# rst-tu-dortmund/mpc_local_planner

Measured on AMD Instinct MI355X. Metric: MPC solves/sec (batched control cycles) at N=50 carlike, higher is better.
Workload: dtype f64

## Files before the change

### mpc_local_planner_amd/csrc/mpc_wave.hpp

```cpp
#pragma once
#include <hip/hip_runtime.h>
#include <type_traits>

#include "mpc_core.hpp"
#include "mpc_dpp_blocks.inc"

#include "mpc_wave_debug.hpp"
#include "mpc_wave_layout.hpp"

namespace mpc {

template <typename T, int MODEL, int EXT = 1, bool OBST = true, int NSC = 0, bool GS = false, bool W2 = false, int SHAPE = 0>
struct IpmWave {
    static constexpr int NSTG = EXT ? NSTG_EXT : NSTG_BASE;
    static constexpr int NTRB = (MODEL == MODEL_KINEMATIC_BICYCLE || MODEL == MODEL_SIMPLE_CAR_FRONT) ? 4 : 3;
    static_assert(NSC == 0 || (EXT == 0 && !OBST), "the fixed layout exists for the headline instantiation only");
    static_assert(!GS || NSC == 0, "the fixed layout keeps its factorisation data in LDS");
    static_assert(!W2 || (!GS && EXT == 0 && !OBST), "the two-wave kernel exists for the headline instantiation in the LDS form only");
    static_assert(SHAPE == 0 || NSC != 0, "a compile-time shape exists for the fixed layout only");
    using LayoutT = typename LayoutOf<NSC, NTRB, NSTG>::type;
    const Problem<T>& P;
    const LayoutT L;
    T* sm;
    T* gmb = nullptr;
    const int lane;
    T x0[3], xf[3], uprev[2], dtprev;
    T mu, rho, delta_last;
    T erho = T(0);
    bool row0_on, fail0;
    bool warm_guess = false;
    mutable int cnt_mult = -1, cnt_bmult = -1;
    mutable T inv_cnt_mult = T(1), inv_cnt_bmult = T(1);
    int nvia = 0;
    int flags;
    MPC_PROF_MEMBERS
    int nfix;
    int my_cand = 0, iter_cap = 0;
    int rows_dropped = 0;
    const double* dual_in = nullptr;
    const int* win_ptr = nullptr;

    __device__ IpmWave(const Problem<T>& p, const WaveLayout& l, T* s, int ln) : P(p), L(LayoutOf<NSC, NTRB, NSTG>::from(l)), sm(s), lane(ln) {}

    __device__ __forceinline__ T& F(int base, int comp, int k) const { return sm[base + comp * L.NS + k]; }
    typedef __attribute__((address_space(1))) T GlbT;
    typedef __attribute__((address_space(1))) char GlbC;
    using SwT = std::conditional_t<GS, GlbT, T>;
    __device__ __forceinline__ GlbT& gw(unsigned word) const { return *(GlbT*)((GlbC*)gmb + (size_t)(word * (unsigned)sizeof(T))); }
    static constexpr int TE_CC = NSTG, TE_Z = NSTG + 3, TNT = GlobalStage::nt(NSTG);
    __device__ __forceinline__ int tile_k(int k) const { return GlobalStage::TILE(L.NS) + ((k + GlobalStage::kGuard) >> 2) * (4 * TNT) + ((k + GlobalStage::kGuard) & 3); }
    __device__ __forceinline__ GlbT& TL_(int e, int k) const { return gw((unsigned)(tile_k(k) + 4 * e)); }
    __device__ __forceinline__ SwT& G_(int i, int k) const { if constexpr (GS) return gw((unsigned)(GlobalStage::GAIN + k * NGAIN + i)); else return sm[L.GAIN + k * NGAIN + i]; }
    static constexpr int NADDv = EXT ? (int)NADD : (int)NADD_BASE;
    __device__ __forceinline__ SwT& S_(int i, int k) const { if constexpr (GS) return TL_(i, k); else return sm[L.STG + k * NSTG + i]; }
    __device__ __forceinline__ T& C_(int i, int k) const { return sm[L.CC + k * 3 + i]; }
    __device__ __forceinline__ SwT& OB_(int which, int m, int k) const {
        if constexpr (GS) return gw((unsigned)(GlobalStage::OBC(L.NS, NSTG) + (which * L.M + m) * L.NS + k)); else return sm[(which == 0 ? L.OG : (which == 1 ? L.OAX : (which == 2 ? L.OAY : L.OHK))) + m * L.NS + k];
    }
    __device__ __forceinline__ SwT& OX_(int which, int m, int k) const {
        if constexpr (GS) return gw((unsigned)(L.OXB + ((which < 4 ? which * L.MT : 4 * L.MT + (which - 4) * L.MD) + m) * L.NS + k));
        else {
            const int base = which == 0 ? L.OAT : (which == 1 ? L.OHXT : (which == 2 ? L.OHYT : (which == 3 ? L.OHTT : (which == 4 ? L.OAD : (which == 5 ? L.OHXD : (which == 6 ? L.OHYD : (which == 7 ? L.OHDD : L.OHTD)))))));
            return sm[base + m * L.NS + k];
        }
    }
    __device__ __forceinline__ GlbT& OE_(int which, int m, int k) const { return gw((unsigned)(L.OEB + (which * L.M + m) * L.NS + k)); }
    __device__ __forceinline__ T& CH_(int i, int k) const { return sm[L.LAMN + i * L.NS + k]; }
    __device__ __forceinline__ T& SCL(int i) const { return sm[L.SC + i]; }
    __device__ __forceinline__ void sync() const { __syncthreads(); }
    __device__ __forceinline__ int nM() const { return OBST ? L.M : 0; }
    __device__ __forceinline__ unsigned short* oi_base() const { return reinterpret_cast<unsigned short*>(sm + L.OI); }
    __device__ __forceinline__ int oi(int m, int k) const { const unsigned v = oi_base()[m * L.NS + k]; return v == 0xffffu ? -1 : (int)v; }
    __device__ __forceinline__ void set_oi(int m, int k, int j) const { oi_base()[m * L.NS + k] = (unsigned short)(j < 0 ? 0xffff : j); }
    __device__ __forceinline__ bool fx(int i) const { if constexpr (SHAPE != 0) return (SHAPE >> i) & 1; else return (flags >> i) & 1; }
    __device__ __forceinline__ bool dtf() const { if constexpr (SHAPE != 0) return (SHAPE >> 3) & 1; else return (flags >> 3) & 1; }
    __device__ __forceinline__ bool dtf_sum() const { return (flags >> 3) & 1; }
    __device__ __forceinline__ bool quad() const { if constexpr (SHAPE != 0) return (SHAPE >> 4) & 1; else return (flags >> 4) & 1; }
    __device__ __forceinline__ bool hasqf() const { if constexpr (SHAPE != 0) return (SHAPE >> 5) & 1; else return (flags >> 5) & 1; }
    __device__ __forceinline__ bool mintime() const { if constexpr (SHAPE != 0) return (SHAPE >> 16) & 1; else return (flags >> 16) & 1; }
    __device__ __forceinline__ bool costx() const { return EXT >= 2; }
    __device__ __forceinline__ void offmul(const T o[3], const T x[3], T y[3]) const {
        y[0] = o[0] * x[1] + o[1] * x[2]; y[1] = o[0] * x[0] + o[2] * x[2]; y[2] = o[1] * x[0] + o[2] * x[1];
    }
    __device__ __forceinline__ T offquad(const T o[3], const T x[3]) const { return T(2) * (o[0] * x[0] * x[1] + o[1] * x[0] * x[2] + o[2] * x[1] * x[2]); }
    __device__ __forceinline__ T fullquad(const T dg[3], const T o[3], const T x[3]) const { return dg[0] * x[0] * x[0] + dg[1] * x[1] * x[1] + dg[2] * x[2] * x[2] + offquad(o, x); }
    __device__ __forceinline__ void xd_final(T alpha, T xd[3]) const {
        for (int i = 0; i < 3; ++i) { xd[i] = fx(i) ? T(0) : xt(i, L.n - 1, alpha) - xf[i]; }
        xd[2] = normalize_theta(xd[2]);
    }
    __device__ __forceinline__ T final_cost_extra(T alpha, T d) const {
        T xd[3]; xd_final(alpha, xd);
        T f = T(0);
        if (hasqf()) f += offquad(P.Qfo, xd);
        if (P.trapz) f += T(0.5) * d * fullquad(P.Q, P.Qo, xd);
        return f;
    }
    __device__ __forceinline__ bool ron(int q) const { if constexpr (SHAPE != 0) return (SHAPE >> (6 + q)) & 1; else return (flags >> (6 + q)) & 1; }
    __device__ __forceinline__ bool ball() const { return EXT && ((flags >> 10) & 1); }
    __device__ __forceinline__ bool via() const { return EXT && ((flags >> 11) & 1); }
    __device__ __forceinline__ bool fpline() const { return EXT && ((flags >> 12) & 1); }
    __device__ __forceinline__ bool intf() const { return EXT && ((flags >> 13) & 1); }
    __device__ __forceinline__ bool dynobs() const { return EXT && ((flags >> 14) & 1); }
    __device__ __forceinline__ bool hessm() const { return EXT && ((flags >> 15) & 1); }
    typedef __attribute__((address_space(3))) T LdsT;
    __device__ __forceinline__ LdsT* lds(int word) const { return (LdsT*)sm + word; }
    typedef __attribute__((address_space(3))) char LdsC;
    __device__ __forceinline__ LdsT* ldsb(unsigned bytes) const { return (LdsT*)((LdsC*)(LdsT*)sm + bytes); }
    __device__ __forceinline__ static LdsT* lds_adv(LdsT* p, int bytes) { return (LdsT*)((LdsC*)p + bytes); }
    __device__ __forceinline__ static const LdsT* lds_adv(const LdsT* p, int bytes) { return (const LdsT*)((const LdsC*)p + bytes); }
    using SwRef = std::conditional_t<GS, unsigned, LdsT*>;
    using SwCRef = std::conditional_t<GS, unsigned, const LdsT*>;
    __device__ __forceinline__ int W_ZC() const { if constexpr (GS) return GlobalStage::ZC; else return L.ZC; }
    __device__ __forceinline__ int STG_W(int i) const { return L.STG + i; }
    __device__ __forceinline__ int GAIN_W(int i) const { if constexpr (GS) return GlobalStage::GAIN + i; else return L.GAIN + i; }
    __device__ __forceinline__ int CC_W(int i) const { return L.CC + i; }
    __device__ __forceinline__ int CH_W(int i) const { return L.LAMN + i * L.NS; }
    static constexpr int STG_S = NSTG, GAIN_S = NGAIN, CC_S = 3;
    __device__ __forceinline__ int ZT_W(int kind) const { return L.ZC + (kind == 1 ? 4 : (kind == 2 ? 3 : 0)); }
    __device__ __forceinline__ static constexpr int zt_entry(int kind) { return TE_Z + (kind == 1 ? 3 : (kind == 2 ? 2 : 0)); }
    __device__ __forceinline__ int GAIN_DUMMY_W() const { if constexpr (GS) return GlobalStage::GAIN + L.NS * NGAIN; else return L.VP; }
    __device__ __forceinline__ T gld(unsigned stage_bytes, unsigned lane_bytes) const { return *(const GlbT*)((const GlbC*)gmb + (size_t)stage_bytes + (size_t)lane_bytes); }
    __device__ __forceinline__ SwRef sw(int word) const { if constexpr (GS) return (unsigned)word * (unsigned)sizeof(T); else return lds(word); }
    __device__ __forceinline__ static constexpr int sw_step(int words) { return GS ? words * (int)sizeof(T) : words; }
    __device__ __forceinline__ T sw_ld(SwCRef p, int i = 0) const { if constexpr (GS) return *(const GlbT*)((const GlbC*)gmb + (size_t)p + (size_t)(i * (int)sizeof(T))); else return p[i]; }
    __device__ __forceinline__ T sw_ld_at(SwCRef p, int step) const { if constexpr (GS) return *(const GlbT*)((const GlbC*)gmb + (size_t)(p + (unsigned)step)); else return p[step]; }
    __device__ __forceinline__ void sw_st(SwRef p, int i, T v) const { if constexpr (GS) *(GlbT*)((GlbC*)gmb + (size_t)p + (size_t)(i * (int)sizeof(T))) = v; else p[i] = v; }

    static constexpr bool kLocalLiterals = NSC != 0 && sizeof(T) == 8;
    static constexpr bool LL = kLocalLiterals;
    int colloc_ = 0;
    __device__ __forceinline__ int colloc() const { if constexpr (kLocalLiterals) return colloc_; else return P.collocation; }
    __device__ __forceinline__ T normalize_theta(T th) const { return mpc::normalize_theta<kLocalLiterals>(th); }
    using LogAccT = LogAcc<T, kLocalLiterals>;

    __device__ __forceinline__ T xt(int i, int k, T alpha) const {
        T x = F(L.X, i, k);
        if (alpha != T(0) && k > 0 && (k < L.n - 1 || !fx(i))) { x += alpha * F(L.DX, i, k); if (i == 2) x = normalize_theta(x); }
        return x;
    }
    __device__ __forceinline__ T ut(int j, int k, T alpha) const {
        T u = F(L.U, j, k);
        if (alpha != T(0)) u += alpha * F(L.DU, j, k);
        return u;
    }

    __device__ __forceinline__ bool row_on(int r, int q) const { return ron(q) && (r > 0 || row0_on); }

    __device__ __forceinline__ T row_val(int UB, T d, int r, int q) const {
        const int n = L.n, j = q & 1;
        T ur = r < n - 1 ? F(UB, j, r) : T(0);
        const T up0 = uprev[0], up1 = uprev[1];
        T um = j ? up1 : up0;
        if (r > 0) um = F(UB, j, r - 1);
        T dtp = r > 0 ? d : dtprev;
        return slot_sign<T>(q) * ((ur - um) - P.rate_lim[q] * dtp);
    }
    __device__ __forceinline__ T row_jdz(int r, int q, T dd) const {
        const int n = L.n, j = q & 1;
        T dur = r < n - 1 ? F(L.DU, j, r) : T(0);
        T dum = r > 0 ? F(L.DU, j, r - 1) : T(0);
        return slot_sign<T>(q) * ((dur - dum) - (r > 0 ? P.rate_lim[q] * dd : T(0)));
    }

    __device__ __forceinline__ T push_interior(T v, T lb, T ub) const {
        T pl = t_min(Algo<T>::bound_push * t_max(T(1), t_abs(lb)), Algo<T>::bound_push * (ub - lb));
        T pu = t_min(Algo<T>::bound_push * t_max(T(1), t_abs(ub)), Algo<T>::bound_push * (ub - lb));
        return t_min(t_max(v, lb + pl), ub - pu);
    }

    __device__ __forceinline__ int local_lane() const { int l = lane; asm volatile("" : "+v"(l)); return l; }
#define MPC_PHASE_LANE const int lane = W2 ? this->local_lane() : this->lane; (void)lane;
    static constexpr bool kUniformScalars = W2 || (EXT == 0 && !OBST && !GS);
    __device__ __forceinline__ static double uni_(double v) { return __hiloint2double(__builtin_amdgcn_readfirstlane(__double2hiint(v)), __builtin_amdgcn_readfirstlane(__double2loint(v))); }
    __device__ __forceinline__ static float uni_(float v) { return __int_as_float(__builtin_amdgcn_readfirstlane(__float_as_int(v))); }
    __device__ __forceinline__ static int uni_(int v) { return __builtin_amdgcn_readfirstlane(v); }
    __device__ __forceinline__ static long long uni_(long long v) { return ((long long)__builtin_amdgcn_readfirstlane((int)(v >> 32)) << 32) | (unsigned)__builtin_amdgcn_readfirstlane((int)v); }
    __device__ __attribute__((noinline)) static T pow_cold(T a, T b) { return t_pow(a, b); }
    __device__ __forceinline__ static T pow_(T a, T b) { if constexpr (W2 || kLocalLiterals) return pow_cold(a, b); else return t_pow(a, b); }
    __device__ __forceinline__ static void U(T& v) { if constexpr (kUniformScalars) v = uni_(v); }
    template <typename... Ts> __device__ __forceinline__ static void U(T& v, Ts&... rest) { U(v); U(rest...); }

#include "mpc_wave_rows.inc"
#include "mpc_wave_passes.inc"
#include "mpc_wave_sweeps.inc"
#include "mpc_wave_pit.inc"
#include "mpc_wave_step.inc"
#include "mpc_wave_solve.inc"
#undef MPC_PHASE_LANE
};

}
```

### mpc_local_planner_amd/csrc/mpc_wave_step.inc

```

    struct Fwd { T hdz, clam, dz2, dphi, a_p, a_d, dzmax, nunu; bool finite; };

    __device__ __forceinline__ void ftb_ratio(T ival, T dval, T& r) const { r = t_max(r, -dval * ival); }
    __device__ __forceinline__ T ftb_alpha(T r, T tau) const { return r > tau ? tau / r : T(1); }

    template <bool REC>
    __device__ __forceinline__ Fwd post_pass(T dd, const T nu[3], T tau, TrialRegs& tr) const {
        MPC_PHASE_LANE
        const int n = L.n;
        const T d = SCL(SC_D);
        T hdz = T(0), clam = T(0), dz2 = T(0), dphi = T(0), r_p = T(0), r_d = T(0), dzmax = T(0);
        if constexpr (REC) {
            trial_setup_states(tr, lane);
            for (int j = 0; j < 2; ++j) { tr.ulb[j] = P.u_lb[j]; tr.uub[j] = P.u_ub[j]; tr.u[j] = tr.du[j] = T(0); }
            for (int q = 0; q < 4; ++q) { tr.on[q] = false; tr.s[q] = T(1); tr.ds[q] = T(0); }
        }
        if (lane == 0) {
            if (dtf()) {
                T dl = d - P.dt_lb, du = P.dt_ub - d;
                T pl = SCL(SC_PDL), pu = SCL(SC_PDU);
                const T idl = t_rcp(dl), idu = t_rcp(du);
                T gb = -mu * idl + mu * idu;
                hdz += gb * dd; dphi += gb * dd;
                ftb_ratio(idl, dd, r_p); ftb_ratio(idu, -dd, r_p);
                ftb_ratio(t_rcp(pl), mu * idl - pl - (pl * idl) * dd, r_d);
                ftb_ratio(t_rcp(pu), mu * idu - pu + (pu * idu) * dd, r_d);
                dz2 += dd * dd; dzmax = t_max(dzmax, t_abs(dd));
            }
            if (mintime()) { hdz += T(n - 1) * dd; dphi += T(n - 1) * dd; }
            if (ball()) {
                const T jdz = ball_jdz(), s = SCL(SC_TS), y = SCL(SC_TY), res = SCL(SC_TG) + s;
                const T is = t_rcp(s);
                const T sig = y * is, ybar = mu * is + sig * res;
                const T ds = -res - jdz, dy = ybar + sig * jdz - y;
                hdz += ybar * jdz;
                dphi -= (mu * is) * ds;
                ftb_ratio(is, ds, r_p);
                ftb_ratio(t_rcp(y), dy, r_d);
            }
        }
        for (int k = lane; k < n; k += kWave) {
            if (k < n - 1) {
                for (int j = 0; j < 2; ++j) {
                    T u = F(L.U, j, k), du_ = F(L.DU, j, k);
                    T dl = u - P.u_lb[j], du = P.u_ub[j] - u;
                    T pl = F(L.PL, j, k), pu = F(L.PU, j, k);
                    const T idl = t_rcp(dl), idu = t_rcp(du);
                    T gbar = mu * idu - mu * idl + (quad() ? T(2) * P.R[j] * u * (intf() ? d : T(1)) : T(0));
                    if (costx() && quad()) gbar += T(2) * P.Ro * F(L.U, 1 - j, k) * (intf() ? d : T(1));
                    hdz += gbar * du_; dphi += gbar * du_;
                    ftb_ratio(idl, du_, r_p); ftb_ratio(idu, -du_, r_p);
                    ftb_ratio(t_rcp(pl), mu * idl - pl - (pl * idl) * du_, r_d);
                    ftb_ratio(t_rcp(pu), mu * idu - pu + (pu * idu) * du_, r_d);
                    dz2 += du_ * du_; dzmax = t_max(dzmax, t_abs(du_));
                    if constexpr (REC) { tr.u[j] = u; tr.du[j] = du_; }
                }
                for (int i = 0; i < 3; ++i) {
                    clam += C_(i, k) * F(L.LAMN, i, k);
                }
                if (intf()) {
                    const T xd0 = F(L.X, 0, k) - xf[0], xd1 = F(L.X, 1, k) - xf[1], xd2 = normalize_theta(F(L.X, 2, k) - xf[2]);
                    const T v = F(L.U, 0, k), w = F(L.U, 1, k);
                    T sc = P.Q[0] * xd0 * xd0 + P.Q[1] * xd1 * xd1 + P.Q[2] * xd2 * xd2 + P.R[0] * v * v + P.R[1] * w * w;
                    if (costx()) {
                        const T xd[3] = {xd0, xd1, xd2};
                        sc += offquad(P.Qo, xd) + T(2) * P.Ro * v * w;
                        if (k == 0 && P.trapz) sc -= T(0.5) * fullquad(P.Q, P.Qo, xd);
                    }
                    hdz += sc * dd; dphi += sc * dd;
                }
            }
            if (k >= 1) {
                T vg[3] = {T(0), T(0), T(0)};
                if (via() && k < n - 1) { T vv; via_terms(k, F(L.X, 0, k), F(L.X, 1, k), F(L.X, 2, k), vv, vg); }
                T gxo[3] = {T(0), T(0), T(0)};
                if (costx()) {
                    if (k < n - 1) {
                        if (quad()) {
                            const T xd[3] = {F(L.X, 0, k) - xf[0], F(L.X, 1, k) - xf[1], normalize_theta(F(L.X, 2, k) - xf[2])};
                            offmul(P.Qo, xd, gxo);
                            for (int i = 0; i < 3; ++i) gxo[i] *= T(2) * (intf() ? d : T(1));
                        }
                    } else {
                        T xdT[3], y3[3]; xd_final(T(0), xdT);
                        if (hasqf()) { offmul(P.Qfo, xdT, y3); for (int i = 0; i < 3; ++i) gxo[i] += T(2) * y3[i]; }
                        if (P.trapz) {
                            offmul(P.Qo, xdT, y3);
                            for (int i = 0; i < 3; ++i) gxo[i] += d * (P.Q[i] * xdT[i] + y3[i]);
                            const T sc = T(0.5) * fullquad(P.Q, P.Qo, xdT);
                            hdz += sc * dd; dphi += sc * dd;
                        }
                    }
                }
                for (int i = 0; i < 3; ++i) {
                    if (k < n - 1 || !fx(i)) {
                        T dx = F(L.DX, i, k);
                        dz2 += dx * dx; dzmax = t_max(dzmax, t_abs(dx));
                        T g = vg[i];
                        if (quad() && k < n - 1) { T xd = F(L.X, i, k) - xf[i]; if (i == 2) xd = normalize_theta(xd); g = T(2) * P.Q[i] * xd * (intf() ? d : T(1)); }
                        else if (k == n - 1 && hasqf()) { T xd = F(L.X, i, k) - xf[i]; if (i == 2) xd = normalize_theta(xd); g += T(2) * P.Qf[i] * xd; }
                        g += gxo[i];
                        hdz += g * dx; dphi += g * dx;
                    }
                }
            }
            for (int q = 0; q < 4; ++q) {
                if (!row_on(k, q)) continue;
                T jdz = row_jdz(k, q, dd);
                T s = F(L.SR, q, k), y = F(L.YR, q, k);
                T res = row_val(L.U, d, k, q) + s;
                const T is = t_rcp(s);
                T sig = y * is;
                T ybar = mu * is + sig * res;
                T ds = -res - jdz;
                T dy = ybar + sig * jdz - y;
                hdz += ybar * jdz;
                dphi -= (mu * is) * ds;
                ftb_ratio(is, ds, r_p);
                ftb_ratio(t_rcp(y), dy, r_d);
                if constexpr (REC) { tr.on[q] = true; tr.s[q] = s; tr.ds[q] = ds; }
            }
            if (nM() > 0 && k >= 1 && k < n - 1) {
                for (int m0 = 0; m0 < nM(); m0 += kRowGroup) {
                RowCache oc;
                ob_load<false>(m0, k, oc);
#pragma unroll
                for (int jm = 0; jm < kRowGroup; ++jm) {
                    const int m = m0 + jm;
                    if (m >= nM()) break;
                    if (oi(m, k) < 0) continue;
                    const T jdz = obst_jdz(k, m, oc.ax[jm], oc.ay[jm]);
                    const T s = F(L.OS, m, k), y = F(L.OY, m, k);
                    if (erho > T(0)) {
                        const T ee = OE_(0, m, k);
                        T ds, de, dy, ybar;
                        elastic_steps(s, y, oc.g[jm], ee, jdz, ds, de, dy, ybar);
                        OE_(1, m, k) = de;
                        hdz += ybar * jdz;
                        dphi += -(mu * t_rcp(s)) * ds - (mu * t_rcp(ee)) * de + erho * de;
                        ftb_ratio(t_rcp(s), ds, r_p); ftb_ratio(t_rcp(ee), de, r_p);
                        ftb_ratio(t_rcp(y), dy, r_d); ftb_ratio(t_rcp(erho - y), -dy, r_d);
                        continue;
                    }
                    const T res = oc.g[jm] + s;
                    const T is = t_rcp(s);
                    const T sig = y * is;
                    const T ybar = mu * is + sig * res;
                    const T ds = -res - jdz;
                    const T dy = ybar + sig * jdz - y;
                    hdz += ybar * jdz;
                    dphi -= (mu * is) * ds;
                    ftb_ratio(is, ds, r_p);
                    ftb_ratio(t_rcp(y), dy, r_d);
                }
                }
            }
        }
        Fwd o;
        if constexpr (kBatchedReductions) {
            T ra[4] = {hdz, clam, r_p, r_d}, rb[3] = {dz2, dphi, dzmax};
            wave_reduce_n<OpSum, OpSum, OpMax, OpMax>(ra);
            wave_reduce_n<OpSum, OpSum, OpMax>(rb);
            o.hdz = ra[0]; o.clam = ra[1]; o.dz2 = rb[0]; o.dphi = rb[1];
            o.a_p = ftb_alpha(ra[2], tau); o.a_d = ftb_alpha(ra[3], tau); o.dzmax = rb[2];
        } else {
        o.hdz = wave_sum(hdz); o.clam = wave_sum(clam); o.dz2 = wave_sum(dz2); o.dphi = wave_sum(dphi);
        o.a_p = ftb_alpha(wave_max(r_p), tau); o.a_d = ftb_alpha(wave_max(r_d), tau); o.dzmax = wave_max(dzmax);
        }
        o.nunu = T(0);
        for (int i = 0; i < 3; ++i) if (fx(i)) o.nunu += nu[i] * nu[i];
        o.finite = t_finite(o.hdz) && t_finite(o.dz2) && t_finite(o.clam);
        return o;
    }

    __device__ __forceinline__ void accept(T alpha, T a_d) const {
        MPC_PHASE_LANE
        const int n = L.n;
        const T kS = T(MPC_LIT(1e10)), ikS = LL ? T(MPC_LIT(1.0 / 1e10)) : T(1) / kS;
        const T d_old = SCL(SC_D), dd = SCL(SC_DD), d_new = d_old + (dtf_sum() ? alpha * dd : T(0));
        T sn[4], yn[4];
        for (int k = ((n - 1) / kWave) * kWave + lane; k >= 0; k -= kWave) {
            const bool act = k < n;
            if (act) {
            for (int q = 0; q < 4; ++q) {
                if (!row_on(k, q)) continue;
                T s = F(L.SR, q, k), y = F(L.YR, q, k);
                T res = row_val(L.U, d_old, k, q) + s;
                T jdz = row_jdz(k, q, dd);
                const T is = t_rcp(s);
                T sig = y * is;
                T ds = -res - jdz;
                T dy = mu * is + sig * res + sig * jdz - y;
                sn[q] = s + alpha * ds;
                T yv = y + a_d * dy;
                const T musn = mu * t_rcp(sn[q]);
                yn[q] = t_min(t_max(yv, musn * ikS), kS * musn);
            }
            if (nM() > 0 && k >= 1 && k < n - 1) {
                for (int m0 = 0; m0 < nM(); m0 += kRowGroup) {
                RowCache oc;
                ob_load<false>(m0, k, oc);
#pragma unroll
                for (int jm = 0; jm < kRowGroup; ++jm) {
                    const int m = m0 + jm;
                    if (m >= nM()) break;
                    if (oi(m, k) < 0) continue;
                    const T jdz = obst_jdz(k, m, oc.ax[jm], oc.ay[jm]);
                    const T s = F(L.OS, m, k), y = F(L.OY, m, k);
                    const T res = oc.g[jm] + s;
                    const T is = t_rcp(s);
                    const T sig = y * is;
                    if (erho > T(0)) {
                        const T ee = OE_(0, m, k);
                        T ds, de, dy, ybar;
                        elastic_steps(s, y, oc.g[jm], ee, jdz, ds, de, dy, ybar);
                        const T so = s + alpha * ds, eo = ee + alpha * de;
                        T yo = y + a_d * dy;
                        const T muso = mu * t_rcp(so), mueo = mu * t_rcp(eo);
                        yo = t_min(t_max(yo, muso * ikS), kS * muso);
                        yo = t_min(t_max(yo, erho - kS * mueo), erho - mueo * ikS);
                        F(L.OS, m, k) = so; F(L.OY, m, k) = yo; OE_(0, m, k) = eo;
                        continue;
                    }
                    const T so = s + alpha * (-res - jdz);
                    T yo = y + a_d * (mu * is + sig * res + sig * jdz - y);
                    const T muso = mu * t_rcp(so);
                    yo = t_min(t_max(yo, muso * ikS), kS * muso);
                    F(L.OS, m, k) = so; F(L.OY, m, k) = yo;
                }
                }
            }
            }
            sync();
            if (act) {
            for (int q = 0; q < 4; ++q) if (row_on(k, q)) { F(L.SR, q, k) = sn[q]; F(L.YR, q, k) = yn[q]; }
            if (k < n - 1) {
                for (int j = 0; j < 2; ++j) {
                    T u = F(L.U, j, k), du_ = F(L.DU, j, k);
                    T dl = u - P.u_lb[j], du = P.u_ub[j] - u;
                    T pl = F(L.PL, j, k), pu = F(L.PU, j, k);
                    const T idl = t_rcp(dl), idu = t_rcp(du);
                    T pln = pl + a_d * (mu * idl - pl - (pl * idl) * du_);
                    T pun = pu + a_d * (mu * idu - pu + (pu * idu) * du_);
                    T un = ut(j, k, alpha);
                    const T mdl = mu * t_rcp(un - P.u_lb[j]), mdu = mu * t_rcp(P.u_ub[j] - un);
                    F(L.PL, j, k) = t_min(t_max(pln, mdl * ikS), kS * mdl);
                    F(L.PU, j, k) = t_min(t_max(pun, mdu * ikS), kS * mdu);
                    F(L.U, j, k) = un;
                }
                for (int i = 0; i < 3; ++i) {
                    T lo = F(L.LAM, i, k);
                    F(L.LAM, i, k) = lo + alpha * (F(L.LAMN, i, k) - lo);
                }
            }
            for (int i = 0; i < 3; ++i) F(L.X, i, k) = xt(i, k, alpha);
            }
        }
        if (lane == 0) {
            if (dtf()) {
                T dl = d_old - P.dt_lb, du = P.dt_ub - d_old;
                T pl = SCL(SC_PDL), pu = SCL(SC_PDU);
                const T idl = t_rcp(dl), idu = t_rcp(du);
                T pln = pl + a_d * (mu * idl - pl - (pl * idl) * dd);
                T pun = pu + a_d * (mu * idu - pu + (pu * idu) * dd);
                const T mdl = mu * t_rcp(d_new - P.dt_lb), mdu = mu * t_rcp(P.dt_ub - d_new);
                SCL(SC_PDL) = t_min(t_max(pln, mdl * ikS), kS * mdl);
                SCL(SC_PDU) = t_min(t_max(pun, mdu * ikS), kS * mdu);
            }
            SCL(SC_D) = d_new;
            if (ball()) {
                const T jdz = ball_jdz(), s = SCL(SC_TS), y = SCL(SC_TY), res = SCL(SC_TG) + s, is = t_rcp(s), sig = y * is;
                const T so = s + alpha * (-res - jdz);
                T yo = y + a_d * (mu * is + sig * res + sig * jdz - y);
                const T muso = mu * t_rcp(so);
                yo = t_min(t_max(yo, muso * ikS), kS * muso);
                SCL(SC_TS) = so; SCL(SC_TY) = yo;
            }
        }
    }

    __device__ __forceinline__ void cold_start() const {
        const int n = L.n;
        const T dth = normalize_theta(xf[2] - x0[2]);
        for (int k = lane; k < n; k += kWave) {
            T fr = T(k) / T(n - 1);
            T xk[3];
            if (k == 0) { xk[0] = x0[0]; xk[1] = x0[1]; xk[2] = x0[2]; }
            else if (k == n - 1) { xk[0] = xf[0]; xk[1] = xf[1]; xk[2] = xf[2]; }
            else {
                xk[0] = x0[0] + fr * (xf[0] - x0[0]);
                xk[1] = x0[1] + fr * (xf[1] - x0[1]);
                xk[2] = normalize_theta(x0[2] + fr * dth);
            }
            for (int i = 0; i < 3; ++i) F(L.X, i, k) = xk[i];
            if (k < n - 1) { F(L.U, 0, k) = T(0); F(L.U, 1, k) = T(0); }
        }
        if (lane == 0) SCL(SC_D) = P.dt_ref;
    }

    __device__ __forceinline__ void seed_start(int kind, T tscale = T(2)) const {
        const int n = L.n;
        const T ddx = xf[0] - x0[0], ddy = xf[1] - x0[1];
        if (kind >= 5) {
            const T sg0 = (kind == 5 || kind == 7) ? T(1) : T(-1), sg1 = (kind == 5 || kind == 8) ? T(1) : T(-1);
            const T dd = sqrt(ddx * ddx + ddy * ddy);
            T s0_, c0_, s1_, c1_;
            t_sincos(x0[2], &s0_, &c0_);
            t_sincos(xf[2], &s1_, &c1_);
            const T m0x = sg0 * tscale * dd * c0_, m0y = sg0 * tscale * dd * s0_, m1x = sg1 * tscale * dd * c1_, m1y = sg1 * tscale * dd * s1_;
            for (int k = lane; k < n; k += kWave) {
                const T t = T(k) / T(n - 1), t2 = t * t, t3 = t2 * t;
                const T h00 = T(2) * t3 - T(3) * t2 + T(1), h10 = t3 - T(2) * t2 + t, h01 = T(-2) * t3 + T(3) * t2, h11 = t3 - t2;
                const T g00 = T(6) * t2 - T(6) * t, g10 = T(3) * t2 - T(4) * t + T(1), g01 = T(-6) * t2 + T(6) * t, g11 = T(3) * t2 - T(2) * t;
                T xk[3];
                if (k == 0) { xk[0] = x0[0]; xk[1] = x0[1]; xk[2] = x0[2]; }
                else if (k == n - 1) { xk[0] = xf[0]; xk[1] = xf[1]; xk[2] = xf[2]; }
                else {
                    xk[0] = h00 * x0[0] + h10 * m0x + h01 * xf[0] + h11 * m1x;
                    xk[1] = h00 * x0[1] + h10 * m0y + h01 * xf[1] + h11 * m1y;
                    const T tx = g00 * x0[0] + g10 * m0x + g01 * xf[0] + g11 * m1x, ty = g00 * x0[1] + g10 * m0y + g01 * xf[1] + g11 * m1y;
                    T th = t_atan2(ty, tx);
                    if ((2 * k < n - 1 ? sg0 : sg1) < T(0)) th = normalize_theta(th + T(3.14159265358979323846));
                    xk[2] = th;
                }
                for (int i = 0; i < 3; ++i) F(L.X, i, k) = xk[i];
                if (k < n - 1) { F(L.U, 0, k) = T(0); F(L.U, 1, k) = T(0); }
            }
            if (lane == 0) SCL(SC_D) = P.dt_ref;
            return;
        }
        T orient = t_atan2(ddy, ddx);
        T s0, c0;
        t_sincos(x0[2], &s0, &c0);
        if (ddx * c0 + ddy * s0 < T(0)) orient = normalize_theta(orient + T(3.14159265358979323846));
        if (kind == 2 || kind == 4) orient = normalize_theta(orient + T(3.14159265358979323846));
        const bool blend = kind >= 3;
        int m = P.cand_blend;
        if (m > (n - 1) / 2) m = (n - 1) / 2;
        const T d0 = normalize_theta(orient - x0[2]), df = normalize_theta(orient - xf[2]);
        for (int k = lane; k < n; k += kWave) {
            const T fr = T(k) / T(n - 1);
            T xk[3];
            if (k == 0) { xk[0] = x0[0]; xk[1] = x0[1]; xk[2] = x0[2]; }
            else if (k == n - 1) { xk[0] = xf[0]; xk[1] = xf[1]; xk[2] = xf[2]; }
            else {
                xk[0] = x0[0] + fr * ddx;
                xk[1] = x0[1] + fr * ddy;
                xk[2] = orient;
                if (blend && k < m) xk[2] = normalize_theta(x0[2] + (T(k) / T(m)) * d0);
                if (blend && n - 1 - k < m) xk[2] = normalize_theta(xf[2] + (T(n - 1 - k) / T(m)) * df);
            }
            for (int i = 0; i < 3; ++i) F(L.X, i, k) = xk[i];
            if (k < n - 1) { F(L.U, 0, k) = T(0); F(L.U, 1, k) = T(0); }
        }
        if (lane == 0) SCL(SC_D) = P.dt_ref;
    }

    __device__ __forceinline__ void store_duals(double* blk) const {
        const int NS = L.NS;
        if (lane == 0) { blk[0] = double(L.n); blk[1] = double(SCL(SC_PDL)); blk[2] = double(SCL(SC_PDU)); blk[3] = ball() ? double(SCL(SC_TY)) : 0.0; }
        for (int e = lane; e < 3 * NS; e += kWave) blk[4 + e] = double(sm[L.LAM + e]);
        for (int e = lane; e < 4 * NS; e += kWave) blk[4 + 3 * NS + e] = double(sm[L.YR + e]);
        for (int e = lane; e < 2 * NS; e += kWave) { blk[4 + 7 * NS + e] = double(sm[L.PL + e]); blk[4 + 9 * NS + e] = double(sm[L.PU + e]); }
    }
    __device__ __forceinline__ void load_duals(const double* blk) const {
        const int n = L.n, NS = L.NS;
        for (int k = lane; k < n; k += kWave) {
            if (k < n - 1) {
                for (int i = 0; i < 3; ++i) F(L.LAM, i, k) = T(blk[4 + i * NS + k]);
                for (int j = 0; j < 2; ++j) {
                    F(L.PL, j, k) = t_max(F(L.PL, j, k), T(blk[4 + 7 * NS + j * NS + k]));
                    F(L.PU, j, k) = t_max(F(L.PU, j, k), T(blk[4 + 9 * NS + j * NS + k]));
                }
            }
            for (int q = 0; q < 4; ++q) if (row_on(k, q)) F(L.YR, q, k) = t_max(F(L.YR, q, k), T(blk[4 + 3 * NS + q * NS + k]));
        }
        if (lane == 0) {
            if (dtf()) { SCL(SC_PDL) = t_max(SCL(SC_PDL), T(blk[1])); SCL(SC_PDU) = t_max(SCL(SC_PDU), T(blk[2])); }
            if (ball()) SCL(SC_TY) = t_max(SCL(SC_TY), T(blk[3]));
        }
    }

    __device__ __forceinline__ void init_point() {
        MPC_PHASE_LANE
        const int n = L.n;
        if (lane == 0) {
            for (int i = 0; i < 3; ++i) {
                F(L.X, i, 0) = x0[i];
                if (fx(i)) F(L.X, i, n - 1) = xf[i];
            }
            if (!dtf()) SCL(SC_D) = P.dt_ref;
        }
        sync();
        T nz = T(0);
        for (int k = lane; k < n - 1; k += kWave) nz += (F(L.U, 0, k) != T(0) || F(L.U, 1, k) != T(0)) ? T(1) : T(0);
        nz = wave_sum(nz);
        const T d0 = SCL(SC_D);
        if (nz == T(0)) {
            for (int k = lane; k < n - 1; k += kWave) {
                T dx = F(L.X, 0, k + 1) - F(L.X, 0, k), dy = F(L.X, 1, k + 1) - F(L.X, 1, k);
                T dth = normalize_theta(F(L.X, 2, k + 1) - F(L.X, 2, k));
                T s, c;
                t_sincos(F(L.X, 2, k), &s, &c);
                T v = (dx * c + dy * s) / d0;
                v = t_min(t_max(v, P.u_lb[0]), P.u_ub[0]);
                T rate = dth / d0, w;
                if (MODEL == MODEL_UNICYCLE) w = rate;
                else {
                    T vv = t_abs(v) > T(1e-3) ? v : (v >= T(0) ? T(1e-3) : T(-1e-3));
                    if (MODEL == MODEL_SIMPLE_CAR) w = t_atan(P.p0 * rate / vv);
                    else if (MODEL == MODEL_SIMPLE_CAR_FRONT) w = t_asin(t_min(T(1), t_max(T(-1), P.p0 * rate / vv)));
                    else { T sb = t_min(T(1), t_max(T(-1), P.p0 * rate / vv)); w = t_atan(t_tan(t_asin(sb)) * (P.p1 + P.p0) / P.p0); }
                }
                w = t_min(t_max(w, P.u_lb[1]), P.u_ub[1]);
                F(L.U, 0, k) = v; F(L.U, 1, k) = w;
            }
            sync();
            if (lane < 2 && ron(lane) && ron(2 + lane)) {
                const int j = lane;
                const T fr = Algo<T>::rate_seed_frac, lo = P.rate_lim[j] * d0 * fr, hi = P.rate_lim[2 + j] * d0 * fr;
                T prev = F(L.U, j, 0);
                if (row0_on) { const T up_ = j ? uprev[1] : uprev[0]; prev = t_min(t_max(prev, up_ + P.rate_lim[j] * dtprev * fr), up_ + P.rate_lim[2 + j] * dtprev * fr); F(L.U, j, 0) = prev; }
                for (int k = 1; k < n - 1; ++k) { prev = t_min(t_max(F(L.U, j, k), prev + lo), prev + hi); F(L.U, j, k) = prev; }
                T nxt = T(0);
                for (int k = n - 2; k >= 0; --k) { nxt = t_min(t_max(F(L.U, j, k), nxt - hi), nxt - lo); F(L.U, j, k) = nxt; }
            }
        }
        sync();
        for (int k = lane; k < n - 1; k += kWave)
            for (int j = 0; j < 2; ++j) F(L.U, j, k) = push_interior(F(L.U, j, k), P.u_lb[j], P.u_ub[j]);
        if (lane == 0 && dtf()) SCL(SC_D) = push_interior(SCL(SC_D), P.dt_lb, P.dt_ub);
        sync();
        if (nM() > 0) { rows_dropped = associate_obstacles(); sync(); }
        if (via()) { associate_via_points(); sync(); }
        const bool dual_ok = dual_in != nullptr && warm_guess && (int)dual_in[0] == n;
        mu = dual_ok ? P.mu_init_dual : (warm_guess ? P.mu_init_warm : P.mu_init); rho = T(0); delta_last = T(0); fail0 = false;
        const T d = SCL(SC_D);
        for (int k = lane; k < n; k += kWave) {
            for (int q = 0; q < 4; ++q) {
                T s = T(1), y = T(0);
                if (row_on(k, q)) { s = t_max(-row_val(L.U, d, k, q), Algo<T>::slack_push); y = mu / s; }
                F(L.SR, q, k) = s; F(L.YR, q, k) = y;
            }
            if (nM() > 0) {
                const T px = F(L.X, 0, k), py = F(L.X, 1, k);
                for (int m = 0; m < nM(); ++m) {
                    T s = T(1), y = T(0), g, a3[3], hk, h3[3];
                    if (k >= 1 && k < n - 1) {
                        if (obst_row3(k, m, px, py, F(L.X, 2, k), g, a3, hk, h3, d)) { s = t_max(-g, Algo<T>::clearance_slack_push); y = mu / s; }
                    } else set_oi(m, k, -1);
                    F(L.OS, m, k) = s; F(L.OY, m, k) = y;
                }
            }
            if (k < n - 1) {
                for (int j = 0; j < 2; ++j) {
                    T u = F(L.U, j, k);
                    F(L.PL, j, k) = mu / (u - P.u_lb[j]);
                    F(L.PU, j, k) = mu / (P.u_ub[j] - u);
                }
                for (int i = 0; i < 3; ++i) F(L.LAM, i, k) = T(0);
            }
        }
        if (lane == 0) {
            SCL(SC_PDL) = dtf() ? mu / (d - P.dt_lb) : T(0);
            SCL(SC_PDU) = dtf() ? mu / (P.dt_ub - d) : T(0);
            if (ball()) {
                T a[3];
                const T s = t_max(-ball_eval(T(0), a), Algo<T>::slack_push);
                SCL(SC_TS) = s; SCL(SC_TY) = mu / s;
            }
        }
        sync();
        if (dual_ok) { load_duals(dual_in); sync(); }
    }
```

Baseline: 360,100.

## Fold dt bound terms into lane-parallel control slot to remove lane-0 serial blocks

For the fixed-layout f64 instantiation, the time-step variable's bound and multiplier work is mapped onto the last grid point's first control slot. Every lane now runs the same straight-line code for control 0 or dt, instead of lane 0 doing a separate serial dt block before and after the per-lane loops. The dt gradient term is broadcast with a lane read, and the dt path uses explicit FMA forms with contraction turned off. This is meant to remove divergent lane-0 sections in the post pass and the update pass. It adds some rounding differences and needs care that the remapped indices match the original dt handling.

```diff
diff --git a/mpc_local_planner_amd/csrc/mpc_wave.hpp b/mpc_local_planner_amd/csrc/mpc_wave.hpp
--- a/mpc_local_planner_amd/csrc/mpc_wave.hpp
+++ b/mpc_local_planner_amd/csrc/mpc_wave.hpp
@@ -133,6 +133,17 @@
     __device__ __forceinline__ T normalize_theta(T th) const { return mpc::normalize_theta<kLocalLiterals>(th); }
     using LogAccT = LogAcc<T, kLocalLiterals>;
 
+    static constexpr bool kStraightPasses = NSC != 0 && sizeof(T) == 8;
+    struct Ctl0 { int u, du, pl, pu; T lb, ub; bool dt; };
+    __device__ __forceinline__ Ctl0 ctl0(int k) const {
+        Ctl0 c;
+        c.dt = dtf() && k == L.n - 1;
+        c.u = c.dt ? L.SC + SC_D : L.U + k; c.du = c.dt ? L.SC + SC_DD : L.DU + k;
+        c.pl = c.dt ? L.SC + SC_PDL : L.PL + k; c.pu = c.dt ? L.SC + SC_PDU : L.PU + k;
+        c.lb = c.dt ? P.dt_lb : P.u_lb[0]; c.ub = c.dt ? P.dt_ub : P.u_ub[0];
+        return c;
+    }
+
     __device__ __forceinline__ T xt(int i, int k, T alpha) const {
         T x = F(L.X, i, k);
         if (alpha != T(0) && k > 0 && (k < L.n - 1 || !fx(i))) { x += alpha * F(L.DX, i, k); if (i == 2) x = normalize_theta(x); }
@@ -169,6 +180,7 @@
     }
 
     __device__ __forceinline__ int local_lane() const { int l = lane; asm volatile("" : "+v"(l)); return l; }
+    __device__ __forceinline__ static T here_(T v) { asm volatile("" : "+v"(v)); return v; }
 #define MPC_PHASE_LANE const int lane = W2 ? this->local_lane() : this->lane; (void)lane;
     static constexpr bool kUniformScalars = W2 || (EXT == 0 && !OBST && !GS);
     __device__ __forceinline__ static double uni_(double v) { return __hiloint2double(__builtin_amdgcn_readfirstlane(__double2hiint(v)), __builtin_amdgcn_readfirstlane(__double2loint(v))); }
diff --git a/mpc_local_planner_amd/csrc/mpc_wave_step.inc b/mpc_local_planner_amd/csrc/mpc_wave_step.inc
--- a/mpc_local_planner_amd/csrc/mpc_wave_step.inc
+++ b/mpc_local_planner_amd/csrc/mpc_wave_step.inc
@@ -15,7 +15,32 @@
             for (int j = 0; j < 2; ++j) { tr.ulb[j] = P.u_lb[j]; tr.uub[j] = P.u_ub[j]; tr.u[j] = tr.du[j] = T(0); }
             for (int q = 0; q < 4; ++q) { tr.on[q] = false; tr.s[q] = T(1); tr.ds[q] = T(0); }
         }
-        if (lane == 0) {
+        T u0 = T(0), du0 = T(0), gbar0 = T(0);
+        if constexpr (kStraightPasses) {
+            static_assert(!kStraightPasses || (NSC > 0 && NSC <= kWave && EXT == 0), "one grid point per lane: lane 0 is grid point 0, and its chains open with dt's terms");
+            T gb_dt = T(0);
+            if (lane < n && (dtf() || lane < n - 1)) {
+                const Ctl0 c = ctl0(lane);
+                T u = sm[c.u], du_ = sm[c.du];
+                T dl = u - c.lb, du = c.ub - u;
+                T pl = sm[c.pl], pu = sm[c.pu];
+                const T idl = t_rcp(dl), idu = t_rcp(du);
+                gbar0 = mu * idu - mu * idl + (quad() ? T(2) * P.R[0] * u * (intf() ? d : T(1)) : T(0));
+                gb_dt = -mu * idl + mu * idu;
+                ftb_ratio(idl, du_, r_p); ftb_ratio(idu, -du_, r_p);
+                ftb_ratio(t_rcp(pl), mu * idl - pl - (pl * idl) * du_, r_d);
+                ftb_ratio(t_rcp(pu), mu * idu - pu + (pu * idu) * du_, r_d);
+                u0 = u; du0 = du_;
+            }
+            const T gb = dtf() ? rd_lane(gb_dt, n - 1) : T(0);
+            if (lane == 0) {
+                if (dtf()) {
+                    hdz += gb * dd; dphi += gb * dd;
+                    dz2 += dd * dd; dzmax = t_max(dzmax, t_abs(dd));
+                }
+                if (mintime()) { hdz += T(n - 1) * dd; dphi += T(n - 1) * dd; }
+            }
+        } else if (lane == 0) {
             if (dtf()) {
                 T dl = d - P.dt_lb, du = P.dt_ub - d;
                 T pl = SCL(SC_PDL), pu = SCL(SC_PDU);
@@ -41,7 +66,13 @@
         }
         for (int k = lane; k < n; k += kWave) {
             if (k < n - 1) {
-                for (int j = 0; j < 2; ++j) {
+                if constexpr (kStraightPasses) {
+                    const T g0 = here_(gbar0), v0 = here_(du0);
+                    hdz += g0 * v0; dphi += g0 * v0;
+                    dz2 += v0 * v0; dzmax = t_max(dzmax, t_abs(v0));
+                    if constexpr (REC) { tr.u[0] = u0; tr.du[0] = v0; }
+                }
+                for (int j = kStraightPasses ? 1 : 0; j < 2; ++j) {
                     T u = F(L.U, j, k), du_ = F(L.DU, j, k);
                     T dl = u - P.u_lb[j], du = P.u_ub[j] - u;
                     T pl = F(L.PL, j, k), pu = F(L.PU, j, k);
@@ -234,8 +265,33 @@
             sync();
             if (act) {
             for (int q = 0; q < 4; ++q) if (row_on(k, q)) { F(L.SR, q, k) = sn[q]; F(L.YR, q, k) = yn[q]; }
+            if constexpr (kStraightPasses) {
+                auto bounded = [&](int wu, int wdu, int wpl, int wpu, T lb, T ub, bool is_dt) {
+#pragma clang fp contract(off)
+                    T u = sm[wu], du_ = sm[wdu];
+                    T dl = u - lb, du = ub - u;
+                    T pl = sm[wpl], pu = sm[wpu];
+                    const T idl = t_rcp(dl), idu = t_rcp(du);
+                    const T al = is_dt ? __builtin_fma(mu, idl, -pl) : mu * idl - pl;
+                    const T au = is_dt ? __builtin_fma(mu, idu, -pu) : mu * idu - pu;
+                    T pln = __builtin_fma(a_d, __builtin_fma(-du_, pl * idl, al), pl);
+                    T pun = __builtin_fma(a_d, __builtin_fma(du_, pu * idu, au), pu);
+                    T un = u;
+                    if (alpha != T(0)) un = __builtin_fma(alpha, du_, u);
+                    un = is_dt ? d_new : un;
+                    const T mdl = mu * t_rcp(un - lb), mdu = mu * t_rcp(ub - un);
+                    sm[wpl] = t_min(t_max(pln, mdl * ikS), kS * mdl);
+                    sm[wpu] = t_min(t_max(pun, mdu * ikS), kS * mdu);
+                    sm[wu] = un;
+                };
+                if (dtf() || k < n - 1) {
+                    const Ctl0 c = ctl0(k);
+                    bounded(c.u, c.du, c.pl, c.pu, c.lb, c.ub, c.dt);
+                }
+                if (k < n - 1) bounded(L.U + L.NS + k, L.DU + L.NS + k, L.PL + L.NS + k, L.PU + L.NS + k, P.u_lb[1], P.u_ub[1], false);
+            }
             if (k < n - 1) {
-                for (int j = 0; j < 2; ++j) {
+                for (int j = kStraightPasses ? 2 : 0; j < 2; ++j) {
                     T u = F(L.U, j, k), du_ = F(L.DU, j, k);
                     T dl = u - P.u_lb[j], du = P.u_ub[j] - u;
                     T pl = F(L.PL, j, k), pu = F(L.PU, j, k);
@@ -256,7 +312,9 @@
             for (int i = 0; i < 3; ++i) F(L.X, i, k) = xt(i, k, alpha);
             }
         }
-        if (lane == 0) {
+        if constexpr (kStraightPasses) {
+            if (lane == 0 && !dtf()) SCL(SC_D) = d_new;
+        } else if (lane == 0) {
             if (dtf()) {
                 T dl = d_old - P.dt_lb, du = P.dt_ub - d_old;
                 T pl = SCL(SC_PDL), pu = SCL(SC_PDU);
```

New measurement: 361,100, median of 2. About the same (+0.3%).
